# dimforge/salva

Measured on NVIDIA H100. Metric: particle-steps/s (DFSPH 3D), higher is better.
Workload: dtype f32

## Files before the change

salva_b200/csrc/sph_engine.cu:

```cuda
#include <cuda_runtime.h>
#include <cub/device/device_radix_sort.cuh>

#include <algorithm>
#include <array>
#include <climits>
#include <cmath>
#include <cstdarg>
#include <cstddef>
#include <cstdio>
#include <cstdlib>
#include <cstring>
#include <memory>
#include <mutex>
#include <string>
#include <type_traits>
#include <utility>
#include <vector>

#include "../../include/sph.h"
#include "sph_kernels.cuh"
#include "sph_shapes.cuh"
#include "sph_passes.cuh"
#include "sph_iisph.cuh"
#include "sph_elasticity.cuh"
// ... 451 lines not shown
    bool staged = true;
    FluidRows rows;
    bool b_dirty = true;
    CellBox b_box = CELL_BOX_EMPTY;
    bool b_sorted_valid = false, b_reused = false;
    unsigned long long bb_contacts = 0;
    int b_sorted_grid[6] = {0, 0, 0, 0, 0, 0};
    BoundaryRows brows;
    bool hb_stale = false;
    std::vector<ColliderRec> colliders;
    DBuf<CellBox> d_cb;
    DBuf<float> d_imp;
    float* h_imp = nullptr;
    DBuf<ContactCollider> d_ccol;
    DBuf<HfGrid> d_chf;
    DBuf<ContactResults> d_cres;
    DBuf<float4> cs_s4, cs_p4;
    DBuf<unsigned long long> cs_key[2];
    DBuf<uint32_t> cs_val[2];
    DBuf<char> cs_tmp;
    uint32_t cap_s = 4096, cap_p = 4096;
    DBuf<float> smp_f, smp_xyz;
    DBuf<unsigned long long> smp_cnt, smp_off, smp_key[2];
    DBuf<int> smp_flag;

    int cur = 0, bcur = 0;
    DBuf<float4> pos[2], vel[2], vc[2], bpos[2], bvel[2];
    DBuf<uint32_t> orig[2], borig[2];
    DBuf<uint32_t> gid[2];
    DBuf<float> press[2];
    DBuf<float4> vs, acc, normals, dbg_acc;
    DBuf<float> dens, alpha, kappa, divv, pred, bvol, bforce;
    DBuf<uint32_t> cid, rank, perm, cstart, bcid, brank, bperm, bstart, scan_aux[3], scan_aux_k[3];
    ListState lists;
    bool unimass = false;
    DBuf<float4> pvx4, pk4;
    DBuf<float2> vyz2;
    Tex tex_pvx, tex_vyz, tex_pk;
    DBuf<float> he_colors, he_gradc;
    DBuf<uint32_t> q_out, q_count;
    DBuf<float> map_pos, map_vel;
    bool in_coupling = false;
    bool in_host_force = false;
    const sph_coupling_manager* coupling = nullptr;
    DBuf<uint32_t> ct_cnt[2], ct_j[2], ct_model[2];
    DBuf<float> ct_w[2], ct_g[2];
    DBuf<float4> xs;
    uint32_t fused_nblk = 0;
    Tex tex_vs;
    DBuf<float> partial;
    DBuf<StepScalars> d_ss;
    StepScalars* h_ss = nullptr;
    DBuf<uint32_t> rows_scratch;
    IisphState iisph;
    ViscosityState visc;

    struct Span { int slot; cudaEvent_t a, b; };
    std::vector<Span> spans;
    size_t n_spans = 0;

    uint32_t stride = 0;
    bool lists_valid = false;
    bool nb_valid = false, nb_pending = false;
    CellBox nb = CELL_BOX_EMPTY;
    std::vector<SinkRec> sinks;
    std::vector<SourceRec> sources;
// ... 317 lines not shown
    o = 0;
    for (auto& b : w->bounds) {
        b.offset = o;
        o += b.n;
    }
    w->B = o;
}

sph_status ensure_fluid_buffers(sph_world* w) {
    size_t N = std::max(w->Ntot, w->N);
    for (int k = 0; k < 2; ++k) {
        if (k == w->protect_buf) continue;
        bool keep = k == w->cur;
        CU(w->pos[k].ensure(N, keep, w->st));
        CU(w->vel[k].ensure(N, keep, w->st));
        CU(w->vc[k].ensure(N, keep, w->st));
        CU(w->orig[k].ensure(N, keep, w->st));
        CU(w->gid[k].ensure(N, keep, w->st));
        if (w->desc.solver == SPH_SOLVER_IISPH) CU(w->press[k].ensure(N, keep, w->st));
    }
    CU(w->vs.ensure(N));
    CU(w->pvx4.ensure(N));
    CU(w->pk4.ensure(N));
    CU(w->vyz2.ensure(N));
    CU(w->acc.ensure(N));
    CU(w->dens.ensure(N + 8));
    CU(w->alpha.ensure(N + 8));
    CU(w->kappa.ensure(N + 8));
    CU(w->divv.ensure(N + 8));
    CU(w->pred.ensure(N + 8));
    CU(w->cid.ensure(N));
    CU(w->rank.ensure(N));
    CU(w->perm.ensure(N));
    w->stride = (uint32_t)((N + 31) / 32 * 32);
    CU(w->lists.ensure(N, w->stride));
    uint32_t nblk = cdiv(std::max<size_t>(N, 1), std::min(PASS_T, NBR_T));
    CU(w->partial.ensure((size_t)(nblk + 3) * std::max<size_t>(1, w->fluids.size())));
    return SPH_OK;
}

sph_status stage_up(sph_world* w) {
    if (!w->staged) return SPH_OK;
    recompute_offsets(w);
    size_t N = w->N;
    w->Ntot = N;
    w->own_begin = 0;
    TRY(ensure_fluid_buffers(w));
    w->vol_all_default = true;
    if (N) {
        const std::vector<float>& vol = w->rows.vol;
        std::vector<float> mass(N);
        std::vector<uint32_t> fid(N);
        bool all_default = true;
        for (size_t g = 0; g < N; ++g) all_default = all_default && vol[g] == w->rows.vol0;
        w->vol_all_default = all_default;
        for (size_t f = 0; f < w->fluids.size(); ++f) {
            bool uniform = w->fluids[f].n > 0;
            for (size_t i = 0; i < w->fluids[f].n; ++i) {
                size_t g = w->fluids[f].offset + i;
                mass[g] = vol[g] * w->fluids[f].density0;
                fid[g] = (uint32_t)f;
                uniform = uniform && vol[g] == vol[w->fluids[f].offset];
            }
            w->fluids[f].uniform_mass = uniform ? mass[w->fluids[f].offset] : 0.f;
        }
        int c = w->cur;
// ... 98 lines not shown
    if (ncell_d > 1.0e9) return w->fail(SPH_ERR_OOM, "dense cell grid too large: %lld x %lld x %lld cells of width h", dims[0], dims[1], dims[2]);
    const int xys = w->slab.active ? 1 : w->xysub;
    if (ncell_d * xys * xys > 2.0e9) return w->fail(SPH_ERR_OOM, "dense cell grid too large: %lld x %lld x %lld cells of width h", dims[0], dims[1], dims[2]);
    size_t ncell = (size_t)dims[0] * dims[1] * dims[2] * xys * xys;
    w->hc.ox = (hb.lo[0] - 1) * xys;
    w->hc.oy = (hb.lo[1] - 1) * xys;
    w->hc.oz = hb.lo[2] - 1;
    w->hc.nx = (int)dims[0] * xys;
    w->hc.ny = (int)dims[1] * xys;
    w->hc.nz = (int)dims[2];
    fill_static_consts(w);
    TRY(upload_consts(w));
    CU(w->cstart.ensure(ncell + 1));
    CU(w->bstart.ensure(ncell + 1));
    w->stats.grid_dims[0] = (uint32_t)dims[0];
    w->stats.grid_dims[1] = (uint32_t)dims[1];
    w->stats.grid_dims[2] = (uint32_t)dims[2];
    *ncell_out = ncell;
    return SPH_OK;
}

sph_status sort_boundaries(sph_world* w, size_t ncell) {
    const size_t B = w->B;
    const int bc = w->bcur;
    const int xys = w->slab.active ? 1 : w->xysub;
    const int gridkey[6] = {w->hc.ox, w->hc.oy, w->hc.oz, w->hc.nx, w->hc.ny, w->hc.nz};
    const bool reuse_b = w->b_sorted_valid && memcmp(gridkey, w->b_sorted_grid, sizeof gridkey) == 0;
    w->b_reused = reuse_b;
    if (!reuse_b) CU(cudaMemsetAsync(w->bstart.p, 0, (ncell + 1) * sizeof(uint32_t), w->st));
    if (B && !reuse_b) {
        if (xys > 1) LAUNCH(k_cell_hist_xy, B, 256, w->bpos[bc].p, (uint32_t)B, w->bcid.p, w->brank.p, w->bstart.p);
        else LAUNCH(k_cell_hist, B, 256, w->bpos[bc].p, (uint32_t)B, w->bcid.p, w->brank.p, w->bstart.p, (const uint32_t*)nullptr, 0u);
        TRY(scan_exclusive(w, w->bstart.p, ncell + 1));
        LAUNCH(k_cell_scatter, B, 256, (uint32_t)B, w->bcid.p, w->brank.p, w->bstart.p, w->bperm.p);
        if (w->desc.deterministic)
            LAUNCH(k_cell_sort, ncell, 256, (uint32_t)ncell, w->bstart.p, w->bperm.p, (const uint32_t*)w->borig[bc].p, (const float4*)nullptr);
        GatherSet g;
        memset(&g, 0, sizeof g);
        g.in4[0] = w->bpos[bc].p; g.out4[0] = w->bpos[bc ^ 1].p;
        g.in4[1] = w->bvel[bc].p; g.out4[1] = w->bvel[bc ^ 1].p;
        g.n4 = 2;
        g.in1[0] = w->borig[bc].p; g.out1[0] = w->borig[bc ^ 1].p;
        g.n1 = 1;
        LAUNCH(k_gather, B, 256, (uint32_t)B, w->bperm.p, g);
        w->bcur = bc ^ 1;
    }
    if (!reuse_b) {
        memcpy(w->b_sorted_grid, gridkey, sizeof gridkey);
        w->b_sorted_valid = true;
    }
    return SPH_OK;
}

sph_status phase_grid(sph_world* w) {
    size_t N = w->Ntot;
    int c = w->cur;
    const uint32_t off = w->slab.active ? w->slab.sort_off : 0u;
    const size_t Nin = w->slab.active ? w->slab.sort_n : N;
    const uint32_t* dead = w->slab.active ? w->slab.flag.p : nullptr;
    const uint32_t n_dead = w->slab.active ? w->slab.sort_dead_n : 0u;
    size_t ncell;
    if (w->cap) {
        CU(cudaMemsetAsync(reinterpret_cast<char*>(w->d_ss.p) + SS_BEGIN(err), 0, SS_END(contacts_f) - SS_BEGIN(err), w->st));
        ncell = (size_t)w->hc.nx * w->hc.ny * w->hc.nz;
    } else {
        StepScalars init{};
        init.grid = CELL_BOX_EMPTY;
        CU(cudaMemcpyAsync(w->d_ss.p, &init, SS_END(contacts_f), cudaMemcpyHostToDevice, w->st));
        CellBox hb;
        if (w->nb_valid && !w->slab.active && N) {
            hb = w->nb;
        } else {
            if (Nin) {
                k_bounds<<<std::min<uint32_t>(cdiv(Nin, 256), 296), 256, 0, w->st>>>(w->pos[c].p + off, (uint32_t)Nin, &w->d_ss.p->grid);
                w->launches++;
            }
            TRY(read_scalars(w, SS_BEGIN(grid), SS_END(grid)));
            CU(cudaStreamSynchronize(w->st));
            hb = w->h_ss->grid;
        }
        w->nb_valid = false;
        if (hb.bad || w->b_box.bad) return w->fail(SPH_ERR_INVALID, "non-finite or out-of-range particle coordinates");
        TRY(grid_size(w, hb, &ncell));
    }
    const int xys = w->slab.active ? 1 : w->xysub;
    CU(cudaMemsetAsync(w->cstart.p, 0, (ncell + 1) * sizeof(uint32_t), w->st));
    if (xys > 1) LAUNCH(k_cell_hist_xy, Nin, 256, w->pos[c].p + off, (uint32_t)Nin, w->cid.p, w->rank.p, w->cstart.p);
    else LAUNCH(k_cell_hist, Nin, 256, w->pos[c].p + off, (uint32_t)Nin, w->cid.p, w->rank.p, w->cstart.p, dead, n_dead);
    TRY(scan_exclusive(w, w->cstart.p, ncell + 1));
    LAUNCH(k_cell_scatter, Nin, 256, (uint32_t)Nin, w->cid.p, w->rank.p, w->cstart.p, w->perm.p);
    if (w->desc.deterministic)
        LAUNCH(k_cell_sort, ncell, 256, (uint32_t)ncell, w->cstart.p, w->perm.p, (const uint32_t*)w->gid[c].p + off,
               w->fluids.size() > 1 ? (const float4*)w->vel[c].p + off : (const float4*)nullptr);
    if (N) {
        GatherSet g;
        memset(&g, 0, sizeof g);
        g.in4[0] = w->pos[c].p + off; g.out4[0] = w->pos[c ^ 1].p;
        g.in4[1] = w->vel[c].p + off; g.out4[1] = w->vel[c ^ 1].p;
        g.in4[2] = w->vc[c].p + off;  g.out4[2] = w->vc[c ^ 1].p;
        g.n4 = 3;
        g.in1[0] = w->orig[c].p + off; g.out1[0] = w->orig[c ^ 1].p;
        g.in1[1] = w->gid[c].p + off; g.out1[1] = w->gid[c ^ 1].p;
        g.n1 = 2;
        if (w->desc.solver == SPH_SOLVER_IISPH) {
            g.in1[2] = reinterpret_cast<const uint32_t*>(w->press[c].p);
            g.out1[2] = reinterpret_cast<uint32_t*>(w->press[c ^ 1].p);
            g.n1 = 3;
        }
        LAUNCH(k_gather_vstar, N, 256, (uint32_t)N, w->perm.p, g, w->vs.p, w->unimass ? w->pvx4.p : nullptr, w->unimass ? w->vyz2.p : nullptr);
        w->cur = c ^ 1;
    }
    TRY(sort_boundaries(w, ncell));
    if (w->cap && !w->b_reused) return w->fail(SPH_ERR_INVALID, "step graph: the boundaries are not sorted on the envelope's grid");
    CU(cudaGetLastError());
    if (w->slab.active) {
        TRY(slab_after_sort(w));
        fill_static_consts(w);
        TRY(upload_consts(w));
    }
    return SPH_OK;
}

sph_status density_args(sph_world* w, DensArgs* D) {
    if (w->unimass) {
        CU(w->tex_vyz.bind(w->vyz2));
        CU(w->tex_pvx.bind(w->pvx4));
// ... 114 lines not shown
    *d = loop_decision(r, i, [&] {
        s = read_error(w, nblk, err);
        return *err;
    });
    return s;
}

bool any_bforce(const sph_world* w) {
    for (auto& b : w->bounds)
        if (b.want_forces) return true;
    return false;
}

#define DISPATCH2(kern, multi, bf, n, threads, ...)                                   \
    do {                                                                              \
        if (multi) {                                                                  \
            if (bf) LAUNCH((kern<true, true>), n, threads, __VA_ARGS__);              \
            else LAUNCH((kern<true, false>), n, threads, __VA_ARGS__);                \
        } else {                                                                      \
            if (bf) LAUNCH((kern<false, true>), n, threads, __VA_ARGS__);             \
            else LAUNCH((kern<false, false>), n, threads, __VA_ARGS__);               \
        }                                                                             \
    } while (0)
#define DISPATCH1(kern, multi, n, threads, ...)                         \
    do {                                                                \
        if (multi) LAUNCH((kern<true>), n, threads, __VA_ARGS__);       \
        else LAUNCH((kern<false>), n, threads, __VA_ARGS__);            \
    } while (0)


sph_status refresh_vstar(sph_world* w) {
    if (!w->slab.active) return SPH_OK;
    if (w->unimass) {
        SlabArray a[3] = {{w->pvx4.p, sizeof(float4)}, {w->vyz2.p, sizeof(float2)}, {w->vs.p, sizeof(float4)}};
        return slab_refresh_n(w, a, 3);
    }
    return slab_refresh(w, w->vs.p, sizeof(float4));
}
sph_status refresh_kappa(sph_world* w) {
    if (!w->slab.active || w->slab.overlap) return SPH_OK;
    if (w->unimass) return slab_refresh(w, w->pk4.p, sizeof(float4));
    return slab_refresh(w, w->kappa.p, sizeof(float));
}

sph_status launch_density_alpha(sph_world* w) {
    size_t N = w->N;
    int c = w->cur, bc = w->bcur;
    const bool multi = w->fluids.size() > 1;
    const Lists L = w->lists.view();
    DISPATCH1(k_density_alpha, multi, N, PASS_T, w->pos[c].p, w->vel[c].p, w->bpos[bc].p, L, w->dens.p, w->alpha.p, &w->d_ss.p->err);
    return SPH_OK;
}
sph_status post_density_refresh(sph_world* w) {
    if (!w->slab.active || !w->N) return SPH_OK;
    if (w->desc.solver == SPH_SOLVER_DFSPH) {
        SlabArray a[2] = {{w->dens.p, sizeof(float)}, {w->unimass ? (void*)w->pk4.p : (void*)w->kappa.p, w->unimass ? sizeof(float4) : sizeof(float)}};
        return slab_refresh_n(w, a, 2);
    }
    return slab_refresh(w, w->dens.p, sizeof(float));
}
#define LAUNCH_R(kern, rg, ...)                                                                   \
    do {                                                                                          \
        if ((rg).count > 0) {                                                                     \
            kern<<<cdiv((rg).count, PASS_T), PASS_T, 0, w->st>>>(__VA_ARGS__, (rg));              \
            w->launches++;                                                                        \
        }                                                                                         \
    } while (0)

// ... 84 lines not shown
    const int n_arrays = (w->slab.active && w->slab.overlap) ? 1 : 0;
    sph_status rs = run_parts(w, a, n_arrays, nblk, [&](Range rg, uint32_t blk) -> sph_status {
        float* partial = w->partial.p + (size_t)blk * nf;
        if (w->unimass) {
            if (predict) {
                LAUNCH_R((k_vel_divergence_u<true>), rg, w->pvx4.p, w->tex_pvx.obj, w->vyz2.p, w->tex_vyz.obj, w->bpos[bc].p, w->bvel[bc].p, L, w->dens.p,
                         w->alpha.p, out, w->pk4.p, partial, w->dt, &w->d_ss.p->err);
            } else if (xsf) {
                const float cf = w->fluids[0].forces[0].d.p[0];
                LAUNCH_R((k_vel_divergence_xsph_u<1>), rg, w->pvx4.p, w->tex_pvx.obj, w->vyz2.p, w->tex_vyz.obj, w->bpos[bc].p, L, w->dens.p, w->alpha.p, out,
                         w->pk4.p, partial, w->xs.p, cf, (const float4*)nullptr, 0.f, 0.f);
            } else if (akf) {
                const AkinciNorms an = akinci_norms(w->h);
                LAUNCH_R((k_vel_divergence_xsph_u<2>), rg, w->pvx4.p, w->tex_pvx.obj, w->vyz2.p, w->tex_vyz.obj, w->bpos[bc].p, L, w->dens.p, w->alpha.p, out,
                         w->pk4.p, partial, w->xs.p, w->fluids[0].forces[0].d.p[0], w->normals.p, an.coh_norm, an.h6_64);
            } else {
                LAUNCH_R((k_vel_divergence_u<false>), rg, w->pvx4.p, w->tex_pvx.obj, w->vyz2.p, w->tex_vyz.obj, w->bpos[bc].p, w->bvel[bc].p, L, w->dens.p,
                         w->alpha.p, out, w->pk4.p, partial, w->dt, &w->d_ss.p->err);
            }
        } else {
            DISPATCH2(k_vel_divergence, multi, predict, rg.count, PASS_T, w->pos[c].p, w->vs.p, w->tex_vs.obj, w->vel[c].p, w->bpos[bc].p, w->bvel[bc].p, L,
                      w->dens.p, w->alpha.p, out, w->kappa.p, partial, w->dt, &w->d_ss.p->err, rg);
        }
        return SPH_OK;
    });
    return rs;
}
sph_status launch_vel_update(sph_world* w, bool pressure, bool normals = false) {
    int c = w->cur, bc = w->bcur;
    const bool multi = w->fluids.size() > 1, bf = any_bforce(w);
    const Lists L = w->lists.view();
    if (w->unimass) CU(w->tex_pk.bind(w->pk4));
    if (normals) CU(w->normals.ensure(std::max(w->Ntot, w->N)));
    SlabArray a[3] = {{w->pvx4.p, sizeof(float4)}, {w->vyz2.p, sizeof(float2)}, {w->vs.p, sizeof(float4)}};
    SlabArray a1[1] = {{w->vs.p, sizeof(float4)}};
    return run_parts(w, w->unimass ? a : a1, w->unimass ? 3 : 1, nullptr, [&](Range rg, uint32_t) -> sph_status {
        if (normals)
            LAUNCH_R((k_vel_update_u<false, false, true>), rg, w->pk4.p, w->tex_pk.obj, w->vel[c].p, w->bpos[bc].p, L, w->vc[c].p, w->vs.p, w->pvx4.p,
                     w->vyz2.p, w->bforce.p, w->inv_dt, w->dens.p, w->normals.p);
        else if (w->unimass)
            DISPATCH2(k_vel_update_u, bf, pressure, rg.count, PASS_T, w->pk4.p, w->tex_pk.obj, w->vel[c].p, w->bpos[bc].p, L, w->vc[c].p, w->vs.p, w->pvx4.p,
                      w->vyz2.p, w->bforce.p, w->inv_dt, (const float*)nullptr, (float4*)nullptr, rg);
        else
            BOOL3(k_vel_update, multi, bf, pressure, rg, w->pos[c].p, w->vel[c].p, w->bpos[bc].p, L, w->kappa.p, w->vc[c].p, w->vs.p, w->bforce.p, w->inv_dt);
        return SPH_OK;
    });
}

struct HostContacts {
    std::vector<uint32_t> offsets, j, model;
    std::vector<float> weight, gradient;
};
sph_status materialise_contacts(sph_world* w, uint32_t f, int which, HostContacts* out) {
    const FluidRec& fl = w->fluids[f];
    const size_t N = w->N, Nf = fl.n;
    const int c = w->cur, bc = w->bcur;
    const uint32_t ob = w->own_begin;
    const uint32_t cap = which ? w->lists.cap_b : w->lists.cap_f;
    const uint32_t* cnt = which ? w->lists.cnt_b.p : w->lists.cnt_f.p;
    CU(w->ct_cnt[which].ensure(N + 1));
    LAUNCH(k_contacts_count, N, 256, (uint32_t)N, w->orig[c].p + ob, cnt + ob, cap, w->ct_cnt[which].p);
    CU(cudaMemsetAsync(w->ct_cnt[which].p + N, 0, sizeof(uint32_t), w->st));
    TRY(scan_exclusive(w, w->ct_cnt[which].p, N + 1));
    std::vector<uint32_t> scan(Nf + 1);
    CU(cudaMemcpyAsync(scan.data(), w->ct_cnt[which].p + fl.offset, (Nf + 1) * sizeof(uint32_t), cudaMemcpyDeviceToHost, w->st));
    uint32_t total = 0;
    CU(cudaMemcpyAsync(&total, w->ct_cnt[which].p + N, sizeof(uint32_t), cudaMemcpyDeviceToHost, w->st));
    CU(cudaStreamSynchronize(w->st));
    CU(w->ct_j[which].ensure(std::max<size_t>(total, 1)));
    CU(w->ct_model[which].ensure(std::max<size_t>(total, 1)));
    CU(w->ct_w[which].ensure(std::max<size_t>(total, 1)));
    CU(w->ct_g[which].ensure(3 * std::max<size_t>(total, 1)));
    OffsetTable tab;
    memset(&tab, 0, sizeof tab);
// ... 174 lines not shown
sph_status timestep_advance(sph_world* w, float remaining) {
    float dt = remaining;
    if (w->cfl_coeff != 0.f) {
        TRY(read_scalars(w, SS_BEGIN(cfl_bits), SS_END(cfl_bits)));
        CU(cudaStreamSynchronize(w->st));
        const uint32_t n = cfl_substeps(__uint_as_float_host(w->h_ss->cfl_bits), remaining, w->desc.particle_radius, w->cfl_coeff, w->min_substeps,
                                        w->max_substeps, (uint32_t)w->substeps.size());
        dt = remaining / (float)n;
    }
    w->dt = dt;
    w->inv_dt = dt == 0.f ? 0.f : 1.0f / dt;
    if (!w->cap) w->substeps.push_back(dt);
    return SPH_OK;
}

sph_status dfsph_fold(sph_world* w, float remaining, const float g[3], uint32_t fold) {
    size_t N = w->N;
    int c = w->cur;
    TRY(slab_wait(w));
    const bool folded = fold & (FOLD_XS | FOLD_AKINCI);
    const float4* xs = folded ? w->xs.p : nullptr;
    const float xs_scale = (fold & FOLD_AKINCI) ? 1.0f : w->inv_dt;
    bool quiet_forces = true;
    for (size_t f = 0; f < w->fluids.size() && quiet_forces; ++f)
        for (const ForceRec& fr : w->fluids[f].forces)
            if (!(folded && f == 0 && &fr == &w->fluids[0].forces[0])) quiet_forces = false;
    if (quiet_forces && w->cfl_coeff == 0.f) {
        TRY(ev_record(w, EV_FOLD));
        TRY(ev_record(w, EV_FORCES));
        TRY(timestep_advance(w, remaining));
        LAUNCH(k_fold_integrate, w->Ntot, 256, w->vel[c].p, w->vc[c].p, w->vs.p, w->acc.p, g[0], g[1], g[2], xs, xs_scale, w->dt,
               w->unimass ? w->pvx4.p : nullptr, w->unimass ? w->vyz2.p : nullptr);
    } else {
        LAUNCH(k_fold_velocities, w->Ntot, 256, w->vel[c].p, w->vc[c].p, w->vs.p, w->acc.p, g[0], g[1], g[2], xs, xs_scale);
        TRY(ev_record(w, EV_FOLD));
        if (!quiet_forces) TRY(phase_forces(w, fold));
        TRY(ev_record(w, EV_FORCES));
        TRY(launch_cfl_max(w, w->vel[c].p, remaining));
        TRY(timestep_advance(w, remaining));
        LAUNCH(k_integrate_acc, N, 256, w->vel[c].p, w->vc[c].p, w->vs.p, w->acc.p, w->dt, w->unimass ? w->pvx4.p : nullptr,
               w->unimass ? w->vyz2.p : nullptr);
    }
    TRY(refresh_vstar(w));
    return ev_record(w, EV_INTEG);
}

struct Cond {
    bool v = false;
    cudaGraphConditionalHandle h = 0;
};
template <class Fn>
sph_status cap_cond(sph_world* w, cudaGraphConditionalHandle h, cudaGraphConditionalNodeType type, Fn body);
sph_status new_handle(sph_world* w, cudaGraphConditionalHandle* h);

sph_status cond_new(sph_world* w, Cond* c) { return w->cap ? new_handle(w, &c->h) : SPH_OK; }

template <class Fn>
sph_status cond(sph_world* w, const Cond& c, cudaGraphConditionalNodeType type, Fn body) {
    if (w->cap) return cap_cond(w, c.h, type, body);
    if (type == cudaGraphCondTypeIf) return c.v ? body() : SPH_OK;
    while (c.v) TRY(body());
    return SPH_OK;
}

sph_status decide(sph_world* w, const LoopRule& r, int i, uint32_t nblk, std::array<Cond*, 5> c) {
    if (w->cap) {
        if (i < 0 || loop_decision(r, (uint32_t)i, [] { return 0.f; }).read) {
// ... 66 lines not shown
    }
    w->stats.n_pressure_iter = w->stats.n_pressure_eval = 0;
    const LoopRule rp = loop_rule(w, false);
    auto press_update = [&]() -> sph_status {
        TRY(refresh_kappa(w));
        TRY(span_begin(w, SP_PUPD));
        TRY(launch_vel_update(w, true));
        return span_end(w);
    };
    auto press_eval = [&]() -> sph_status {
        TRY(span_begin(w, SP_PRED));
        TRY(launch_vel_divergence(w, true, &nblk));
        return span_end(w);
    };
    if (rp.maxit > 0) {
        Cond more, tail;
        TRY(cond_new(w, &more));
        TRY(cond_new(w, &tail));
        TRY(press_eval());
        TRY(decide(w, rp, 0, nblk, {nullptr, &more, &tail}));
        TRY(cond(w, more, cudaGraphCondTypeWhile, [&] {
            TRY(press_update());
            TRY(press_eval());
            return decide(w, rp, -1, nblk, {nullptr, &more, &tail});
        }));
        TRY(cond(w, tail, cudaGraphCondTypeIf, press_update));
    }
    TRY(ev_record(w, EV_PRESS));
    TRY(slab_wait(w));
    {
        CellBox* next = &w->d_ss.p->next;
        if (w->cap) k_bounds_init<<<1, 1, 0, w->st>>>(next);
        else CU(cudaMemcpyAsync(next, &CELL_BOX_EMPTY, sizeof(CellBox), cudaMemcpyHostToDevice, w->st));
        LAUNCH(k_update_positions, N, 256, w->pos[c].p, w->vs.p, w->dt, w->slab.active ? nullptr : next);
        w->nb_pending = !w->slab.active;
    }
    CU(cudaGetLastError());
    return SPH_OK;
}

void stats_merge(sph_step_stats& t, const sph_step_stats& s) {
    sph_step_stats m = s;
    m.step_ms = t.step_ms + s.step_ms;
    m.grid_ms = t.grid_ms + s.grid_ms;
    m.neighbors_ms = t.neighbors_ms + s.neighbors_ms;
    m.density_ms = t.density_ms + s.density_ms;
    m.divergence_ms = t.divergence_ms + s.divergence_ms;
    m.nonpressure_ms = t.nonpressure_ms + s.nonpressure_ms;
    m.pressure_ms = t.pressure_ms + s.pressure_ms;
    m.integrate_ms = t.integrate_ms + s.integrate_ms;
    m.n_divergence_iter = t.n_divergence_iter + s.n_divergence_iter;
    m.n_pressure_iter = t.n_pressure_iter + s.n_pressure_iter;
    m.n_divergence_eval = t.n_divergence_eval + s.n_divergence_eval;
    m.n_pressure_eval = t.n_pressure_eval + s.n_pressure_eval;
    m.max_neighbors = std::max(t.max_neighbors, s.max_neighbors);
    t = m;
}

sph_status world_substep(sph_world* w, float remaining, const float g[3], const sph_coupling_manager* coupling, bool colliders,
                         bool b_uploaded) {
    const size_t N = w->N, k = w->substeps.size();
    for (ColliderRec& c : w->colliders) c.impulse_pending = false;
    if (colliders) TRY(colliders_update(w, b_uploaded));
    TRY(phase_grid(w));
    w->grid_ready = true;
    w->ever_stepped = true;
    if (colliders && any_contact(w)) TRY(colliders_contact(w));
// ... 1329 lines not shown
```

salva_b200/csrc/sph_kernels.cuh:

```cuda
#pragma once
#include <cuda_runtime.h>
#include <stdint.h>
#include <algorithm>
#include <climits>

namespace sphk {

constexpr int MAX_FLUIDS = 16;
constexpr int MAX_BOUNDARIES = 64;
constexpr float F32_EPS = 1.1920929e-07f;

struct FluidParams {
    float density0;
    uint32_t memberships, filter;
    float mass;
};
struct BoundaryParams {
    uint32_t memberships, filter;
};
struct Consts {
    float h, inv_h, h2;
    float sigma;
    float dsigma;
    float dsigma6;
// ... 271 lines not shown

__device__ __forceinline__ bool groups_test(uint32_t m1, uint32_t f1, uint32_t m2, uint32_t f2) {
    return (m1 & f2) != 0 && (m2 & f1) != 0;
}

__device__ __forceinline__ float warp_sum(float v) {
#pragma unroll
    for (int o = 16; o > 0; o >>= 1) v += __shfl_xor_sync(0xffffffffu, v, o);
    return v;
}
__device__ __forceinline__ float block_sum(float v, float* sm ) {
    v = warp_sum(v);
    int lane = threadIdx.x & 31, wid = threadIdx.x >> 5;
    __syncthreads();
    if (lane == 0) sm[wid] = v;
    __syncthreads();
    if (wid == 0) {
        int nw = (blockDim.x + 31) >> 5;
        v = lane < nw ? sm[lane] : 0.f;
        v = warp_sum(v);
    }
    return v;
}

__global__ void k_bounds(const float4* __restrict__ pos, uint32_t n, CellBox* __restrict__ out) {
    CellBox b = CELL_BOX_EMPTY;
    for (uint32_t i = blockIdx.x * blockDim.x + threadIdx.x; i < n; i += gridDim.x * blockDim.x) {
        const float4 p = pos[i];
        cell_box_add(b, p.x, p.y, p.z, C.h);
    }
    cell_box_commit_block(b, out);
}

__global__ void k_cell_hist(const float4* __restrict__ pos, uint32_t n, uint32_t* __restrict__ cid, uint32_t* __restrict__ rank,
                            uint32_t* __restrict__ count, const uint32_t* __restrict__ dead, uint32_t n_dead) {
    uint32_t i = blockIdx.x * blockDim.x + threadIdx.x;
    if (i >= n) return;
    if (dead && i < n_dead && dead[i]) {
        cid[i] = 0xFFFFFFFFu;
        return;
    }
    float4 p = pos[i];
    uint32_t id = (uint32_t)cell_id(cell_coord(p.x), cell_coord(p.y), cell_coord(p.z));
    cid[i] = id;
    rank[i] = atomicAdd(&count[id], 1u);
}

__global__ void k_cell_hist_xy(const float4* __restrict__ pos, uint32_t n, uint32_t* __restrict__ cid, uint32_t* __restrict__ rank,
                               uint32_t* __restrict__ count) {
    uint32_t i = blockIdx.x * blockDim.x + threadIdx.x;
    if (i >= n) return;
    float4 p = pos[i];
    uint32_t id = (uint32_t)cell_id(abin(p.x, C.xysub, C.xysub_f), abin(p.y, C.xysub, C.xysub_f), cell_coord(p.z));
    cid[i] = id;
    rank[i] = atomicAdd(&count[id], 1u);
}

__global__ void k_cell_scatter(uint32_t n, const uint32_t* __restrict__ cid, const uint32_t* __restrict__ rank,
                               const uint32_t* __restrict__ start, uint32_t* __restrict__ perm) {
    uint32_t i = blockIdx.x * blockDim.x + threadIdx.x;
    if (i >= n) return;
    const uint32_t c = cid[i];
    if (c == 0xFFFFFFFFu) return;
    perm[start[c] + rank[i]] = i;
}

__device__ __forceinline__ unsigned long long sort_key(uint32_t src, const uint32_t* __restrict__ gid, const float4* __restrict__ vel) {
    if (!gid) return src;
    const uint32_t f = vel ? fid_of(vel[src]) : 0u;
    return ((unsigned long long)f << 32) | gid[src];
}
__global__ void k_cell_sort(uint32_t ncell, const uint32_t* __restrict__ start, uint32_t* __restrict__ perm, const uint32_t* __restrict__ gid,
                            const float4* __restrict__ vel) {
    uint32_t c = blockIdx.x * blockDim.x + threadIdx.x;
    if (c >= ncell) return;
    uint32_t s = start[c], e = start[c + 1];
    for (uint32_t a = s + 1; a < e; ++a) {
        const uint32_t v = perm[a];
        const unsigned long long kv = sort_key(v, gid, vel);
        uint32_t b = a;
        while (b > s) {
            const uint32_t u = perm[b - 1];
            const unsigned long long ku = sort_key(u, gid, vel);
            if (ku < kv || (ku == kv && u < v)) break;
            perm[b] = u;
            --b;
        }
        perm[b] = v;
    }
}

struct GatherSet {
    const float4* in4[6];
    float4* out4[6];
    const uint32_t* in1[4];
    uint32_t* out1[4];
    int n4, n1;
};
__global__ void k_gather(uint32_t n, const uint32_t* __restrict__ perm, GatherSet g) {
    uint32_t s = blockIdx.x * blockDim.x + threadIdx.x;
    if (s >= n) return;
    uint32_t src = perm[s];
#pragma unroll
    for (int a = 0; a < 6; ++a)
        if (a < g.n4) g.out4[a][s] = g.in4[a][src];
#pragma unroll
    for (int a = 0; a < 4; ++a)
        if (a < g.n1) g.out1[a][s] = g.in1[a][src];
}

constexpr int SCAN_T = 256, SCAN_I = 8, SCAN_B = SCAN_T * SCAN_I;
__global__ void k_scan_block(const uint32_t* __restrict__ in, uint32_t* __restrict__ out, uint32_t n, uint32_t* __restrict__ block_sums) {
    __shared__ uint32_t warp_tot[SCAN_T / 32];
    uint32_t base = blockIdx.x * SCAN_B + threadIdx.x * SCAN_I;
    uint32_t v[SCAN_I];
    uint32_t tsum = 0;
#pragma unroll
    for (int k = 0; k < SCAN_I; ++k) {
        v[k] = (base + k < n) ? in[base + k] : 0u;
        tsum += v[k];
    }
// ... 433 lines not shown
__global__ void k_reduce_partials(const float* __restrict__ partial, uint32_t nblocks, int n_fluids, float* __restrict__ out) {
    __shared__ float sm[32];
    int f = blockIdx.x;
    float s = 0.f;
    for (uint32_t b = threadIdx.x; b < nblocks; b += blockDim.x) s += partial[(size_t)b * n_fluids + f];
    s = block_sum(s, sm);
    if (threadIdx.x == 0) out[f] = s;
}

#ifndef SPH_PASS_T
#define SPH_PASS_T 128
#endif
#ifndef SPH_PASS_MINB
#define SPH_PASS_MINB 9
#endif
#ifndef SPH_FORCE_MINB
#define SPH_FORCE_MINB 8
#endif
constexpr int PASS_T = SPH_PASS_T;

__global__ void k_gather_vstar(uint32_t n, const uint32_t* __restrict__ perm, GatherSet g, float4* __restrict__ vs, float4* __restrict__ pvx,
                               float2* __restrict__ vyz) {
    uint32_t s = blockIdx.x * blockDim.x + threadIdx.x;
    if (s >= n) return;
    const uint32_t src = perm[s];
    const float4 p = g.in4[0][src], v = g.in4[1][src], c = g.in4[2][src];
    g.out4[0][s] = p;
    g.out4[1][s] = v;
    g.out4[2][s] = c;
#pragma unroll
    for (int a = 0; a < 4; ++a)
        if (a < g.n1) g.out1[a][s] = g.in1[a][src];
    const float sx = v.x + c.x, sy = v.y + c.y, sz = v.z + c.z;
    vs[s] = make_float4(sx, sy, sz, 0.f);
    if (pvx) {
        pvx[s] = make_float4(p.x, p.y, p.z, sx);
        vyz[s] = make_float2(sy, sz);
    }
}

__global__ void k_fold_velocities(float4* __restrict__ vel, float4* __restrict__ vc, const float4* __restrict__ vs, float4* __restrict__ acc, float gx, float gy,
                                  float gz, const float4* __restrict__ xs, float scale) {
    uint32_t i = blockIdx.x * blockDim.x + threadIdx.x;
    if (i >= C.n_fluid) return;
    float4 v = vel[i], s = vs[i];
    vel[i] = make_float4(s.x, s.y, s.z, v.w);
    vc[i] = make_float4(0.f, 0.f, 0.f, 0.f);
    float ax = gx, ay = gy, az = gz;
    if (xs) {
        float4 f = xs[i];
        ax = __fadd_rn(gx, __fmul_rn(f.x, scale));
        ay = __fadd_rn(gy, __fmul_rn(f.y, scale));
        az = __fadd_rn(gz, __fmul_rn(f.z, scale));
    }
    acc[i] = make_float4(ax, ay, az, 0.f);
}
__global__ void k_fold_integrate(float4* __restrict__ vel, float4* __restrict__ vc, float4* __restrict__ vs, float4* __restrict__ acc, float gx, float gy,
                                 float gz, const float4* __restrict__ xs, float scale, float dt_new, float4* __restrict__ pvx, float2* __restrict__ vyz) {
    uint32_t i = blockIdx.x * blockDim.x + threadIdx.x;
    if (i >= C.n_fluid) return;
    const float4 v = vel[i], s = vs[i];
    const float4 nv = make_float4(s.x, s.y, s.z, v.w);
    vel[i] = nv;
    const bool owned = i >= C.i_begin && i < C.i_begin + C.n_owned;
    float ax = gx, ay = gy, az = gz;
    if (xs) {
        const float4 f = xs[i];
        ax = __fadd_rn(gx, __fmul_rn(f.x, scale));
        ay = __fadd_rn(gy, __fmul_rn(f.y, scale));
        az = __fadd_rn(gz, __fmul_rn(f.z, scale));
    }
    acc[i] = make_float4(ax, ay, az, 0.f);
    if (!owned) {
        vc[i] = make_float4(0.f, 0.f, 0.f, 0.f);
        return;
    }
    const float cx = __fmul_rn(ax, dt_new), cy = __fmul_rn(ay, dt_new), cz = __fmul_rn(az, dt_new);
    vc[i] = make_float4(cx, cy, cz, 0.f);
    const float sx = nv.x + cx, sy = nv.y + cy, sz = nv.z + cz;
    vs[i] = make_float4(sx, sy, sz, 0.f);
    if (pvx) {
        pvx[i].w = sx;
        vyz[i] = make_float2(sy, sz);
    }
}
__global__ void k_set_gravity(const float4* __restrict__ vel, float4* __restrict__ vs, float4* __restrict__ acc, float gx, float gy, float gz) {
    SPH_OWNED_INDEX(i)
    float4 v = vel[i];
    vs[i] = make_float4(v.x, v.y, v.z, 0.f);
    acc[i] = make_float4(gx, gy, gz, 0.f);
}

__global__ void k_integrate_acc(const float4* __restrict__ vel, float4* __restrict__ vc, float4* __restrict__ vs, const float4* __restrict__ acc, float dt,
                                float4* __restrict__ pvx, float2* __restrict__ vyz) {
    SPH_OWNED_INDEX(i)
    float4 a = acc[i], c = vc[i], v = vel[i];
    c.x += a.x * dt; c.y += a.y * dt; c.z += a.z * dt;
    vc[i] = c;
    float sx = v.x + c.x, sy = v.y + c.y, sz = v.z + c.z;
    vs[i] = make_float4(sx, sy, sz, 0.f);
    if (pvx) {
        pvx[i].w = sx;
        vyz[i] = make_float2(sy, sz);
    }
}

__global__ void k_cfl_max(const float4* __restrict__ vel, const float4* __restrict__ acc, float remaining, unsigned int* __restrict__ out) {
    const uint32_t i = blockIdx.x * blockDim.x + threadIdx.x;
    unsigned int bits = 0u;
    if (i < C.n_owned) {
        const float4 v = vel[C.i_begin + i], a = acc[C.i_begin + i];
        const float x = __fadd_rn(v.x, __fmul_rn(a.x, remaining));
        const float y = __fadd_rn(v.y, __fmul_rn(a.y, remaining));
        const float z = __fadd_rn(v.z, __fmul_rn(a.z, remaining));
        bits = __float_as_uint(__fadd_rn(__fadd_rn(__fmul_rn(x, x), __fmul_rn(y, y)), __fmul_rn(z, z)));
    }
    bits = __reduce_max_sync(0xffffffffu, bits);
    if ((threadIdx.x & 31u) == 0u && bits) atomicMax(out, bits);
}

__global__ void k_update_positions(float4* __restrict__ pos, const float4* __restrict__ vs, float dt, CellBox* __restrict__ bounds_out) {
    uint32_t i = blockIdx.x * blockDim.x + threadIdx.x;
    const bool valid = i < C.n_owned;
    i += C.i_begin;
    CellBox b = CELL_BOX_EMPTY;
    if (valid) {
        float4 p = pos[i], v = vs[i];
        p.x += v.x * dt; p.y += v.y * dt; p.z += v.z * dt;
        pos[i] = p;
        if (bounds_out) cell_box_add(b, p.x, p.y, p.z, C.h);
    }
    if (!bounds_out) return;
    cell_box_commit_block(b, bounds_out);
}

__device__ __forceinline__ float powi3(float x) { return x * x * x; }
__device__ __forceinline__ float cohesion_kernel(float r, float coh_norm, float h6_64) {
    float hr = powi3(C.h - r) * powi3(r);
    float c = r <= C.h * 0.5f ? 2.0f * hr - h6_64 : (r <= C.h ? hr : 0.f);
    return coh_norm * c;
}

__device__ __forceinline__ float adhesion_kernel(float r, float adh_norm) {
    if (r > C.h * 0.5f && r <= C.h) {
        float x = fmaxf(-4.0f * r * r / C.h + 6.0f * r - 2.0f * C.h, 0.f);
        return adh_norm * sqrtf(sqrtf(x));
    }
    return 0.f;
}

__global__ void k_iota(uint32_t n, uint32_t* __restrict__ a) {
    uint32_t s = blockIdx.x * blockDim.x + threadIdx.x;
    if (s < n) a[s] = s;
}
struct SlabOut {
    float4 *pos, *vel, *vc;
    uint32_t* gid;
};
__device__ __forceinline__ uint32_t warp_append(bool pred, uint32_t* counter) {
    const unsigned m = __ballot_sync(0xffffffffu, pred);
// ... 306 lines not shown
```

salva_b200/csrc/sph_passes.cuh:

```cuda
#pragma once
#include <type_traits>

#include "sph_kernels.cuh"

namespace sphk {

struct NoAux {};

template <class F>
__device__ __forceinline__ auto call_gather(F& f, uint32_t j, int u) {
    if constexpr (std::is_invocable_v<F, uint32_t, int>) return f(j, u);
    else return f(j);
}

struct Range {
    uint32_t begin, count;
};

template <bool W, bool G, class LP, class LD, class FF>
__device__ __forceinline__ void for_fluid_contacts_g(uint32_t i, const float4& pi, const Lists& L, LP ldpos, LD ld, FF ff) {
    const uint32_t n = L.fluid_count(i);
    const uint32_t nq = (n + 3u) >> 2;
    uint4 J = nq ? L.group(i, 0) : make_uint4(i, i, i, i);
    for (uint32_t q = 0; q < nq; ++q) {
// ... 364 lines not shown
                 float4* __restrict__ acc, float* __restrict__ bforce, float gamma, float adh, float coh_norm, float h6_64, float adh_norm) {
    SPH_OWNED_INDEX(i)
    const float4 a = pvx[i];
    const float4 ni = nr4[i];
    const float rho0 = C.fluids[0].density0, mass = C.fluids[0].mass;
    const float4 pi = make_float4(a.x, a.y, a.z, mass);
    const float rho_i = ni.w;
    float ax = 0.f, ay = 0.f, az = 0.f;
    if (gamma != 0.f)
        for_fluid_contacts_g<false, false>(
            i, pi, L, [&](uint32_t j) { return tex1Dfetch<float4>(tpvx, (int)j); }, [&](uint32_t j) { return __ldg(&nr4[j]); },
            [&](uint32_t, const Pair& p, const float4&, const float4& nj) {
                akinci_contact(p, ni, rho_i, nj, nj.w, mass, gamma, rho0, coh_norm, h6_64, ax, ay, az);
            });
    if (adh != 0.f)
        for_boundary_contacts<false, false>(i, pi, L, bpos, [&](uint32_t j, const Pair& p, const float4& pj) {
            float ad = p.d2 > F32_EPS * F32_EPS ? adhesion_kernel(p.r, adh_norm) / p.r : 0.f;
            float c = ad * adh * (pj.w * rho0);
            ax -= c * p.dx; ay -= c * p.dy; az -= c * p.dz;
            if (BFORCE) {
                atomicAdd(&bforce[3 * (size_t)j + 0], c * p.dx * mass);
                atomicAdd(&bforce[3 * (size_t)j + 1], c * p.dy * mass);
                atomicAdd(&bforce[3 * (size_t)j + 2], c * p.dz * mass);
            }
        });
    float4 o = acc[i];
    o.x += ax; o.y += ay; o.z += az;
    acc[i] = o;
}

template <bool BFORCE, bool PRESSURE, bool NORMALS = false>
__global__ void __launch_bounds__(PASS_T, NORMALS && SPH_GENERIC_KERNELS ? SPH_FORCE_MINB : SPH_PASS_MINB)
k_vel_update_u(const float4* __restrict__ pk4, cudaTextureObject_t tpk, const float4* __restrict__ vel, const float4* __restrict__ bpos, Lists L,
               float4* __restrict__ vc, float4* __restrict__ vs, float4* __restrict__ pvx, float2* __restrict__ vyz, float* __restrict__ bforce,
               float inv_dt, const float* __restrict__ dens, float4* __restrict__ nr4, Range rg) {
    uint32_t i = blockIdx.x * blockDim.x + threadIdx.x;
    if (i >= rg.count) return;
    i += rg.begin;
    const float4 a = pk4[i];
    const float4 pi = make_float4(a.x, a.y, a.z, 0.f);
    const float ki = a.w;
    const float4 v = vel[i];
    const float rho0 = C.fluids[0].density0, mass = C.fluids[0].mass;
    const float scale = (PRESSURE ? inv_dt : 1.0f) * mass;
    float ax = 0.f, ay = 0.f, az = 0.f, nx = 0.f, ny = 0.f, nz = 0.f;
    for_fluid_grads(
        i, pi, L, [&](uint32_t j, int u) { return !(u & 1) ? tex1Dfetch<float4>(tpk, (int)j) : __ldg(&pk4[j]); },
        [&](uint32_t j) {
            if constexpr (NORMALS) return __ldg(&dens[j]);
            else return NoAux{};
        },
        [&](uint32_t, const Pair& p, const float4& pj, auto rho_j) {
            float c = (ki + pj.w) * scale * p.g;
            ax = fmaf(c, p.dx, ax); ay = fmaf(c, p.dy, ay); az = fmaf(c, p.dz, az);
            if constexpr (NORMALS) {
                float cn = p.g * (mass / rho_j);
                nx = fmaf(cn, p.dx, nx); ny = fmaf(cn, p.dy, ny); nz = fmaf(cn, p.dz, nz);
            }
        });
    if (NORMALS) nr4[i] = make_float4(nx * C.h, ny * C.h, nz * C.h, dens[i]);
    if (!PRESSURE || ki > 0.f) {
        const float bscale = PRESSURE ? inv_dt : 1.0f;
        for_boundary_contacts<false, true>(i, pi, L, bpos, [&](uint32_t j, const Pair& p, const float4& pj) {
            float c = ki * pj.w * rho0 * bscale * p.g;
            ax = fmaf(c, p.dx, ax); ay = fmaf(c, p.dy, ay); az = fmaf(c, p.dz, az);
            if (BFORCE) {
                float s = c * inv_dt * mass;
                atomicAdd(&bforce[3 * (size_t)j + 0], s * p.dx);
                atomicAdd(&bforce[3 * (size_t)j + 1], s * p.dy);
                atomicAdd(&bforce[3 * (size_t)j + 2], s * p.dz);
            }
        });
    }
    float4 c4 = vc[i];
    c4.x -= ax; c4.y -= ay; c4.z -= az;
    vc[i] = c4;
    const float sx = v.x + c4.x, sy = v.y + c4.y, sz = v.z + c4.z;
    vs[i] = make_float4(sx, sy, sz, 0.f);
    pvx[i] = make_float4(a.x, a.y, a.z, sx);
    vyz[i] = make_float2(sy, sz);
}

struct VelRho {
    float4 v;
    float rho;
};
template <bool MULTI, bool BFORCE>
__global__ void __launch_bounds__(PASS_T, SPH_FORCE_MINB)
k_force_xsph(const float4* __restrict__ pos, const float4* __restrict__ vel, const float4* __restrict__ bpos, const float4* __restrict__ bvel, Lists L,
             const float* __restrict__ dens, float4* __restrict__ acc, float* __restrict__ bforce, uint32_t which, float cf, float cb, float inv_dt) {
    SPH_OWNED_INDEX(i)
    float4 vi = vel[i];
    if (MULTI && fid_of(vi) != which) return;
    float4 pi = pos[i];
    float rho0 = C.fluids[which].density0;
    float fx = 0.f, fy = 0.f, fz = 0.f, bx = 0.f, by = 0.f, bz = 0.f;
    if (cf != 0.f)
        for_fluid_contacts<true, false>(
            i, pi, L, pos, [&](uint32_t j) { return VelRho{__ldg(&vel[j]), __ldg(&dens[j])}; },
            [&](uint32_t, const Pair& p, const float4& pj, const VelRho& a) {
                if (MULTI && fid_of(a.v) != which) return;
                float c = cf * p.w * pj.w / a.rho;
                fx = fmaf(c, a.v.x - vi.x, fx); fy = fmaf(c, a.v.y - vi.y, fy); fz = fmaf(c, a.v.z - vi.z, fz);
            });
    if (cb != 0.f) {
        float rho_i = dens[i];
        for_boundary_contacts<true, false>(i, pi, L, bpos, [&](uint32_t j, const Pair& p, const float4& pj) {
            float4 vj = __ldg(&bvel[j]);
            float c = cb * p.w * pj.w * rho0 / rho_i;
            float dx = c * (vj.x - vi.x), dy = c * (vj.y - vi.y), dz = c * (vj.z - vi.z);
            bx += dx; by += dy; bz += dz;
// ... 221 lines not shown
```

Before: 979.4 million.

## Drop redundant vs writes in unimass path, warp-aggregate cell histogram, precompute sort keys

In the uniform-mass path, the v* array is no longer written. Consumers such as the fold, integrate and position update kernels now rebuild v* from the packed pvx4/vyz2 arrays, and the slab refresh no longer exchanges vs. This cuts one float4 store per particle in several per-iteration kernels. The cell histogram now groups equal cell ids within a warp using match_any and issues one atomic per group. The deterministic per-cell insertion sort reads keys precomputed during the scatter instead of regathering gid and vel. The risk is any remaining reader of vs in unimass mode that was not updated, which would see stale data.

```diff
diff --git a/salva_b200/csrc/sph_engine.cu b/salva_b200/csrc/sph_engine.cu
--- a/salva_b200/csrc/sph_engine.cu
+++ b/salva_b200/csrc/sph_engine.cu
@@ -507,6 +507,7 @@
     DBuf<float4> vs, acc, normals, dbg_acc;
     DBuf<float> dens, alpha, kappa, divv, pred, bvol, bforce;
     DBuf<uint32_t> cid, rank, perm, cstart, bcid, brank, bperm, bstart, scan_aux[3], scan_aux_k[3];
+    DBuf<unsigned long long> skey;
     ListState lists;
     bool unimass = false;
     DBuf<float4> pvx4, pk4;
@@ -890,6 +891,7 @@
     CU(w->cid.ensure(N));
     CU(w->rank.ensure(N));
     CU(w->perm.ensure(N));
+    if (w->desc.deterministic) CU(w->skey.ensure(N));
     w->stride = (uint32_t)((N + 31) / 32 * 32);
     CU(w->lists.ensure(N, w->stride));
     uint32_t nblk = cdiv(std::max<size_t>(N, 1), std::min(PASS_T, NBR_T));
@@ -1054,9 +1056,11 @@
         if (xys > 1) LAUNCH(k_cell_hist_xy, B, 256, w->bpos[bc].p, (uint32_t)B, w->bcid.p, w->brank.p, w->bstart.p);
         else LAUNCH(k_cell_hist, B, 256, w->bpos[bc].p, (uint32_t)B, w->bcid.p, w->brank.p, w->bstart.p, (const uint32_t*)nullptr, 0u);
         TRY(scan_exclusive(w, w->bstart.p, ncell + 1));
-        LAUNCH(k_cell_scatter, B, 256, (uint32_t)B, w->bcid.p, w->brank.p, w->bstart.p, w->bperm.p);
-        if (w->desc.deterministic)
-            LAUNCH(k_cell_sort, ncell, 256, (uint32_t)ncell, w->bstart.p, w->bperm.p, (const uint32_t*)w->borig[bc].p, (const float4*)nullptr);
+        const bool det = w->desc.deterministic;
+        if (det) CU(w->skey.ensure(B));
+        LAUNCH(k_cell_scatter, B, 256, (uint32_t)B, w->bcid.p, w->brank.p, w->bstart.p, w->bperm.p, (const uint32_t*)w->borig[bc].p,
+               (const float4*)nullptr, det ? w->skey.p : nullptr);
+        if (det) LAUNCH(k_cell_sort, ncell, 256, (uint32_t)ncell, w->bstart.p, w->bperm.p, w->skey.p);
         GatherSet g;
         memset(&g, 0, sizeof g);
         g.in4[0] = w->bpos[bc].p; g.out4[0] = w->bpos[bc ^ 1].p;
@@ -1110,10 +1114,11 @@
     if (xys > 1) LAUNCH(k_cell_hist_xy, Nin, 256, w->pos[c].p + off, (uint32_t)Nin, w->cid.p, w->rank.p, w->cstart.p);
     else LAUNCH(k_cell_hist, Nin, 256, w->pos[c].p + off, (uint32_t)Nin, w->cid.p, w->rank.p, w->cstart.p, dead, n_dead);
     TRY(scan_exclusive(w, w->cstart.p, ncell + 1));
-    LAUNCH(k_cell_scatter, Nin, 256, (uint32_t)Nin, w->cid.p, w->rank.p, w->cstart.p, w->perm.p);
-    if (w->desc.deterministic)
-        LAUNCH(k_cell_sort, ncell, 256, (uint32_t)ncell, w->cstart.p, w->perm.p, (const uint32_t*)w->gid[c].p + off,
-               w->fluids.size() > 1 ? (const float4*)w->vel[c].p + off : (const float4*)nullptr);
+    const bool det = w->desc.deterministic;
+    if (det) CU(w->skey.ensure(Nin));
+    LAUNCH(k_cell_scatter, Nin, 256, (uint32_t)Nin, w->cid.p, w->rank.p, w->cstart.p, w->perm.p, (const uint32_t*)w->gid[c].p + off,
+           w->fluids.size() > 1 ? (const float4*)w->vel[c].p + off : (const float4*)nullptr, det ? w->skey.p : nullptr);
+    if (det) LAUNCH(k_cell_sort, ncell, 256, (uint32_t)ncell, w->cstart.p, w->perm.p, w->skey.p);
     if (N) {
         GatherSet g;
         memset(&g, 0, sizeof g);
@@ -1294,8 +1299,8 @@
 sph_status refresh_vstar(sph_world* w) {
     if (!w->slab.active) return SPH_OK;
     if (w->unimass) {
-        SlabArray a[3] = {{w->pvx4.p, sizeof(float4)}, {w->vyz2.p, sizeof(float2)}, {w->vs.p, sizeof(float4)}};
-        return slab_refresh_n(w, a, 3);
+        SlabArray a[2] = {{w->pvx4.p, sizeof(float4)}, {w->vyz2.p, sizeof(float2)}};
+        return slab_refresh_n(w, a, 2);
     }
     return slab_refresh(w, w->vs.p, sizeof(float4));
 }
@@ -1446,14 +1451,14 @@
     const Lists L = w->lists.view();
     if (w->unimass) CU(w->tex_pk.bind(w->pk4));
     if (normals) CU(w->normals.ensure(std::max(w->Ntot, w->N)));
-    SlabArray a[3] = {{w->pvx4.p, sizeof(float4)}, {w->vyz2.p, sizeof(float2)}, {w->vs.p, sizeof(float4)}};
+    SlabArray a[2] = {{w->pvx4.p, sizeof(float4)}, {w->vyz2.p, sizeof(float2)}};
     SlabArray a1[1] = {{w->vs.p, sizeof(float4)}};
-    return run_parts(w, w->unimass ? a : a1, w->unimass ? 3 : 1, nullptr, [&](Range rg, uint32_t) -> sph_status {
+    return run_parts(w, w->unimass ? a : a1, w->unimass ? 2 : 1, nullptr, [&](Range rg, uint32_t) -> sph_status {
         if (normals)
-            LAUNCH_R((k_vel_update_u<false, false, true>), rg, w->pk4.p, w->tex_pk.obj, w->vel[c].p, w->bpos[bc].p, L, w->vc[c].p, w->vs.p, w->pvx4.p,
+            LAUNCH_R((k_vel_update_u<false, false, true>), rg, w->pk4.p, w->tex_pk.obj, w->vel[c].p, w->bpos[bc].p, L, w->vc[c].p, w->pvx4.p,
                      w->vyz2.p, w->bforce.p, w->inv_dt, w->dens.p, w->normals.p);
         else if (w->unimass)
-            DISPATCH2(k_vel_update_u, bf, pressure, rg.count, PASS_T, w->pk4.p, w->tex_pk.obj, w->vel[c].p, w->bpos[bc].p, L, w->vc[c].p, w->vs.p, w->pvx4.p,
+            DISPATCH2(k_vel_update_u, bf, pressure, rg.count, PASS_T, w->pk4.p, w->tex_pk.obj, w->vel[c].p, w->bpos[bc].p, L, w->vc[c].p, w->pvx4.p,
                       w->vyz2.p, w->bforce.p, w->inv_dt, (const float*)nullptr, (float4*)nullptr, rg);
         else
             BOOL3(k_vel_update, multi, bf, pressure, rg, w->pos[c].p, w->vel[c].p, w->bpos[bc].p, L, w->kappa.p, w->vc[c].p, w->vs.p, w->bforce.p, w->inv_dt);
@@ -1694,7 +1699,8 @@
         LAUNCH(k_fold_integrate, w->Ntot, 256, w->vel[c].p, w->vc[c].p, w->vs.p, w->acc.p, g[0], g[1], g[2], xs, xs_scale, w->dt,
                w->unimass ? w->pvx4.p : nullptr, w->unimass ? w->vyz2.p : nullptr);
     } else {
-        LAUNCH(k_fold_velocities, w->Ntot, 256, w->vel[c].p, w->vc[c].p, w->vs.p, w->acc.p, g[0], g[1], g[2], xs, xs_scale);
+        LAUNCH(k_fold_velocities, w->Ntot, 256, w->vel[c].p, w->vc[c].p, w->vs.p, w->acc.p, g[0], g[1], g[2], xs, xs_scale,
+               w->unimass ? (const float4*)w->pvx4.p : nullptr, w->unimass ? (const float2*)w->vyz2.p : nullptr);
         TRY(ev_record(w, EV_FOLD));
         if (!quiet_forces) TRY(phase_forces(w, fold));
         TRY(ev_record(w, EV_FORCES));
@@ -1827,7 +1833,8 @@
         CellBox* next = &w->d_ss.p->next;
         if (w->cap) k_bounds_init<<<1, 1, 0, w->st>>>(next);
         else CU(cudaMemcpyAsync(next, &CELL_BOX_EMPTY, sizeof(CellBox), cudaMemcpyHostToDevice, w->st));
-        LAUNCH(k_update_positions, N, 256, w->pos[c].p, w->vs.p, w->dt, w->slab.active ? nullptr : next);
+        LAUNCH(k_update_positions, N, 256, w->pos[c].p, w->vs.p, w->unimass ? (const float4*)w->pvx4.p : nullptr,
+               w->unimass ? (const float2*)w->vyz2.p : nullptr, w->dt, w->slab.active ? nullptr : next);
         w->nb_pending = !w->slab.active;
     }
     CU(cudaGetLastError());
diff --git a/salva_b200/csrc/sph_kernels.cuh b/salva_b200/csrc/sph_kernels.cuh
--- a/salva_b200/csrc/sph_kernels.cuh
+++ b/salva_b200/csrc/sph_kernels.cuh
@@ -327,61 +327,91 @@
     cell_box_commit_block(b, out);
 }
 
+__device__ __forceinline__ uint32_t warp_cell_rank(uint32_t id, bool live, uint32_t* __restrict__ count) {
+    const uint32_t lane = threadIdx.x & 31u;
+    const uint32_t peers = __match_any_sync(0xffffffffu, live ? id : 0xFFFFFFFFu);
+    const uint32_t leader = __ffs(peers) - 1u;
+    uint32_t base = 0u;
+    if (live && lane == leader) base = atomicAdd(&count[id], (uint32_t)__popc(peers));
+    base = __shfl_sync(0xffffffffu, base, leader);
+    return base + __popc(peers & ((1u << lane) - 1u));
+}
+
 __global__ void k_cell_hist(const float4* __restrict__ pos, uint32_t n, uint32_t* __restrict__ cid, uint32_t* __restrict__ rank,
                             uint32_t* __restrict__ count, const uint32_t* __restrict__ dead, uint32_t n_dead) {
-    uint32_t i = blockIdx.x * blockDim.x + threadIdx.x;
-    if (i >= n) return;
-    if (dead && i < n_dead && dead[i]) {
-        cid[i] = 0xFFFFFFFFu;
-        return;
-    }
-    float4 p = pos[i];
-    uint32_t id = (uint32_t)cell_id(cell_coord(p.x), cell_coord(p.y), cell_coord(p.z));
+    const uint32_t i = blockIdx.x * blockDim.x + threadIdx.x;
+    const bool in = i < n;
+    const bool live = in && !(dead && i < n_dead && dead[i]);
+    uint32_t id = 0xFFFFFFFFu;
+    if (live) {
+        const float4 p = pos[i];
+        id = (uint32_t)cell_id(cell_coord(p.x), cell_coord(p.y), cell_coord(p.z));
+    }
+    const uint32_t r = warp_cell_rank(id, live, count);
+    if (!in) return;
     cid[i] = id;
-    rank[i] = atomicAdd(&count[id], 1u);
+    if (live) rank[i] = r;
 }
 
 __global__ void k_cell_hist_xy(const float4* __restrict__ pos, uint32_t n, uint32_t* __restrict__ cid, uint32_t* __restrict__ rank,
                                uint32_t* __restrict__ count) {
-    uint32_t i = blockIdx.x * blockDim.x + threadIdx.x;
-    if (i >= n) return;
-    float4 p = pos[i];
-    uint32_t id = (uint32_t)cell_id(abin(p.x, C.xysub, C.xysub_f), abin(p.y, C.xysub, C.xysub_f), cell_coord(p.z));
+    const uint32_t i = blockIdx.x * blockDim.x + threadIdx.x;
+    const bool live = i < n;
+    uint32_t id = 0xFFFFFFFFu;
+    if (live) {
+        const float4 p = pos[i];
+        id = (uint32_t)cell_id(abin(p.x, C.xysub, C.xysub_f), abin(p.y, C.xysub, C.xysub_f), cell_coord(p.z));
+    }
+    const uint32_t r = warp_cell_rank(id, live, count);
+    if (!live) return;
     cid[i] = id;
-    rank[i] = atomicAdd(&count[id], 1u);
-}
-
+    rank[i] = r;
+}
+
+__device__ __forceinline__ unsigned long long sort_key(uint32_t src, const uint32_t* __restrict__ gid, const float4* __restrict__ vel) {
+    const uint32_t f = vel ? fid_of(vel[src]) : 0u;
+    return ((unsigned long long)f << 32) | gid[src];
+}
 __global__ void k_cell_scatter(uint32_t n, const uint32_t* __restrict__ cid, const uint32_t* __restrict__ rank,
-                               const uint32_t* __restrict__ start, uint32_t* __restrict__ perm) {
+                               const uint32_t* __restrict__ start, uint32_t* __restrict__ perm, const uint32_t* __restrict__ gid = nullptr,
+                               const float4* __restrict__ vel = nullptr, unsigned long long* __restrict__ key = nullptr) {
     uint32_t i = blockIdx.x * blockDim.x + threadIdx.x;
     if (i >= n) return;
     const uint32_t c = cid[i];
     if (c == 0xFFFFFFFFu) return;
-    perm[start[c] + rank[i]] = i;
-}
-
-__device__ __forceinline__ unsigned long long sort_key(uint32_t src, const uint32_t* __restrict__ gid, const float4* __restrict__ vel) {
-    if (!gid) return src;
-    const uint32_t f = vel ? fid_of(vel[src]) : 0u;
-    return ((unsigned long long)f << 32) | gid[src];
-}
-__global__ void k_cell_sort(uint32_t ncell, const uint32_t* __restrict__ start, uint32_t* __restrict__ perm, const uint32_t* __restrict__ gid,
-                            const float4* __restrict__ vel) {
+    const uint32_t d = start[c] + rank[i];
+    perm[d] = i;
+    if (key) key[d] = sort_key(i, gid, vel);
+}
+
+__global__ void k_cell_sort(uint32_t ncell, const uint32_t* __restrict__ start, uint32_t* __restrict__ perm, unsigned long long* __restrict__ key) {
     uint32_t c = blockIdx.x * blockDim.x + threadIdx.x;
     if (c >= ncell) return;
-    uint32_t s = start[c], e = start[c + 1];
+    const uint32_t s = start[c], e = start[c + 1];
+    if (e - s < 2u) return;
+    unsigned long long kt = key[s];
+    uint32_t ut = perm[s];
     for (uint32_t a = s + 1; a < e; ++a) {
         const uint32_t v = perm[a];
-        const unsigned long long kv = sort_key(v, gid, vel);
-        uint32_t b = a;
+        const unsigned long long kv = key[a];
+        if (kt < kv || (kt == kv && ut < v)) {
+            kt = kv;
+            ut = v;
+            continue;
+        }
+        perm[a] = ut;
+        key[a] = kt;
+        uint32_t b = a - 1;
         while (b > s) {
             const uint32_t u = perm[b - 1];
-            const unsigned long long ku = sort_key(u, gid, vel);
+            const unsigned long long ku = key[b - 1];
             if (ku < kv || (ku == kv && u < v)) break;
             perm[b] = u;
+            key[b] = ku;
             --b;
         }
         perm[b] = v;
+        key[b] = kv;
     }
 }
 
@@ -881,18 +911,25 @@
     for (int a = 0; a < 4; ++a)
         if (a < g.n1) g.out1[a][s] = g.in1[a][src];
     const float sx = v.x + c.x, sy = v.y + c.y, sz = v.z + c.z;
-    vs[s] = make_float4(sx, sy, sz, 0.f);
     if (pvx) {
         pvx[s] = make_float4(p.x, p.y, p.z, sx);
         vyz[s] = make_float2(sy, sz);
-    }
+    } else {
+        vs[s] = make_float4(sx, sy, sz, 0.f);
+    }
+}
+
+__device__ __forceinline__ float4 load_vstar(uint32_t i, const float4* __restrict__ vs, const float4* __restrict__ pvx, const float2* __restrict__ vyz) {
+    if (!pvx) return vs[i];
+    const float2 b = vyz[i];
+    return make_float4(pvx[i].w, b.x, b.y, 0.f);
 }
 
 __global__ void k_fold_velocities(float4* __restrict__ vel, float4* __restrict__ vc, const float4* __restrict__ vs, float4* __restrict__ acc, float gx, float gy,
-                                  float gz, const float4* __restrict__ xs, float scale) {
+                                  float gz, const float4* __restrict__ xs, float scale, const float4* __restrict__ pvx, const float2* __restrict__ vyz) {
     uint32_t i = blockIdx.x * blockDim.x + threadIdx.x;
     if (i >= C.n_fluid) return;
-    float4 v = vel[i], s = vs[i];
+    const float4 v = vel[i], s = load_vstar(i, vs, pvx, vyz);
     vel[i] = make_float4(s.x, s.y, s.z, v.w);
     vc[i] = make_float4(0.f, 0.f, 0.f, 0.f);
     float ax = gx, ay = gy, az = gz;
@@ -908,7 +945,15 @@
                                  float gz, const float4* __restrict__ xs, float scale, float dt_new, float4* __restrict__ pvx, float2* __restrict__ vyz) {
     uint32_t i = blockIdx.x * blockDim.x + threadIdx.x;
     if (i >= C.n_fluid) return;
-    const float4 v = vel[i], s = vs[i];
+    const float4 v = vel[i];
+    float4 s, r;
+    if (pvx) {
+        r = pvx[i];
+        const float2 b = vyz[i];
+        s = make_float4(r.w, b.x, b.y, 0.f);
+    } else {
+        s = vs[i];
+    }
     const float4 nv = make_float4(s.x, s.y, s.z, v.w);
     vel[i] = nv;
     const bool owned = i >= C.i_begin && i < C.i_begin + C.n_owned;
@@ -927,10 +972,11 @@
     const float cx = __fmul_rn(ax, dt_new), cy = __fmul_rn(ay, dt_new), cz = __fmul_rn(az, dt_new);
     vc[i] = make_float4(cx, cy, cz, 0.f);
     const float sx = nv.x + cx, sy = nv.y + cy, sz = nv.z + cz;
-    vs[i] = make_float4(sx, sy, sz, 0.f);
     if (pvx) {
-        pvx[i].w = sx;
+        pvx[i] = make_float4(r.x, r.y, r.z, sx);
         vyz[i] = make_float2(sy, sz);
+    } else {
+        vs[i] = make_float4(sx, sy, sz, 0.f);
     }
 }
 __global__ void k_set_gravity(const float4* __restrict__ vel, float4* __restrict__ vs, float4* __restrict__ acc, float gx, float gy, float gz) {
@@ -947,10 +993,11 @@
     c.x += a.x * dt; c.y += a.y * dt; c.z += a.z * dt;
     vc[i] = c;
     float sx = v.x + c.x, sy = v.y + c.y, sz = v.z + c.z;
-    vs[i] = make_float4(sx, sy, sz, 0.f);
     if (pvx) {
         pvx[i].w = sx;
         vyz[i] = make_float2(sy, sz);
+    } else {
+        vs[i] = make_float4(sx, sy, sz, 0.f);
     }
 }
 
@@ -968,13 +1015,15 @@
     if ((threadIdx.x & 31u) == 0u && bits) atomicMax(out, bits);
 }
 
-__global__ void k_update_positions(float4* __restrict__ pos, const float4* __restrict__ vs, float dt, CellBox* __restrict__ bounds_out) {
+__global__ void k_update_positions(float4* __restrict__ pos, const float4* __restrict__ vs, const float4* __restrict__ pvx, const float2* __restrict__ vyz,
+                                   float dt, CellBox* __restrict__ bounds_out) {
     uint32_t i = blockIdx.x * blockDim.x + threadIdx.x;
     const bool valid = i < C.n_owned;
     i += C.i_begin;
     CellBox b = CELL_BOX_EMPTY;
     if (valid) {
-        float4 p = pos[i], v = vs[i];
+        float4 p = pos[i];
+        const float4 v = load_vstar(i, vs, pvx, vyz);
         p.x += v.x * dt; p.y += v.y * dt; p.z += v.z * dt;
         pos[i] = p;
         if (bounds_out) cell_box_add(b, p.x, p.y, p.z, C.h);
diff --git a/salva_b200/csrc/sph_passes.cuh b/salva_b200/csrc/sph_passes.cuh
--- a/salva_b200/csrc/sph_passes.cuh
+++ b/salva_b200/csrc/sph_passes.cuh
@@ -420,7 +420,7 @@
 template <bool BFORCE, bool PRESSURE, bool NORMALS = false>
 __global__ void __launch_bounds__(PASS_T, NORMALS && SPH_GENERIC_KERNELS ? SPH_FORCE_MINB : SPH_PASS_MINB)
 k_vel_update_u(const float4* __restrict__ pk4, cudaTextureObject_t tpk, const float4* __restrict__ vel, const float4* __restrict__ bpos, Lists L,
-               float4* __restrict__ vc, float4* __restrict__ vs, float4* __restrict__ pvx, float2* __restrict__ vyz, float* __restrict__ bforce,
+               float4* __restrict__ vc, float4* __restrict__ pvx, float2* __restrict__ vyz, float* __restrict__ bforce,
                float inv_dt, const float* __restrict__ dens, float4* __restrict__ nr4, Range rg) {
     uint32_t i = blockIdx.x * blockDim.x + threadIdx.x;
     if (i >= rg.count) return;
@@ -464,7 +464,6 @@
     c4.x -= ax; c4.y -= ay; c4.z -= az;
     vc[i] = c4;
     const float sx = v.x + c4.x, sy = v.y + c4.y, sz = v.z + c4.z;
-    vs[i] = make_float4(sx, sy, sz, 0.f);
     pvx[i] = make_float4(a.x, a.y, a.z, sx);
     vyz[i] = make_float2(sy, sz);
 }
```

Measured after the change: 1.013 billion, median of 6. +3.4%, better.
